# olga24912/lodestar

Hardware: AMD Instinct MI355X
Metric: verified signature sets/sec (node) (higher is better)
Workload: dtype u32/u64 (28-bit-limb Montgomery integer arithmetic); 1 GPU; C2 gossip attestation flood: 16384 single-pubkey sets per GPU, 1 set per batchable job; pk_mode=device table, sig_encoding=compressed 96 B, distinct_messages=16384, group_sets=1024, group_policy=0, inflight=32, slots=3, hw_queues=4, merge_sets=131072, pipeline_depth=3, parallelism=shard-by-job x1 (in-process devices), no collective

## Files before the change

### include/blsgpu.h

```cpp
#ifndef BLSGPU_H
#define BLSGPU_H

#include <stdint.h>

#ifdef __cplusplus
extern "C" {
#endif

#define BLSGPU_ABI_VERSION 8

#define BLSGPU_JOB_BATCHABLE 1u
#define BLSGPU_JOB_URGENT 2u

enum blsgpu_code {
  BLSGPU_OK = 0,
  BLSGPU_BAD_ENCODING = 1,
  BLSGPU_POINT_NOT_ON_CURVE = 2,
  BLSGPU_POINT_NOT_IN_GROUP = 3,
  BLSGPU_AGGR_TYPE_MISMATCH = 4,
  BLSGPU_VERIFY_FAIL = 5,
  BLSGPU_PK_IS_INFINITY = 6,
  BLSGPU_BAD_SCALAR = 7,
  BLSGPU_INVALID_SIZE = 8,
  BLSGPU_EMPTY_AGGREGATE = 9,
// ... 67 lines not shown
                                const uint8_t* sigs, uint32_t sig_stride, const uint32_t* sig_len,
                                uint32_t flags, uint8_t* out, uint32_t out_len, int8_t* status,
                                uint32_t* first_bad);
uint32_t blsgpu_sig_agg_lanes(uint32_t n_groups, uint32_t n_sigs);

int blsgpu_randomness_words(uint32_t n, uint64_t seed, uint64_t* words);

int blsgpu_aggregate_with_randomness(blsgpu_ctx* ctx, uint32_t n_groups, const uint32_t* group_first,
                                     const uint8_t* pk_bytes, const uint32_t* pk_index, const uint8_t* sigs,
                                     uint32_t sig_stride, const uint32_t* sig_len, uint64_t seed, uint8_t* out_pk,
                                     uint32_t out_pk_len, uint8_t* out_sig, uint32_t out_sig_len, int8_t* status,
                                     uint32_t* first_bad);
uint32_t blsgpu_awr_lanes(uint32_t n_groups, uint32_t n_sets);

#define BLSGPU_SAME_LANE_FORMS 1u

typedef struct blsgpu_same_message_stats {
  uint32_t groups_accepted;
  uint32_t groups_retried;
  uint32_t retry_sets;
  uint32_t unique_messages;
  uint32_t form;
  double device_ms;
} blsgpu_same_message_stats;

int blsgpu_verify_same_message(blsgpu_ctx* ctx, uint32_t n_groups, const uint32_t* group_first,
                               const uint8_t* msgs , const uint8_t* pk_bytes,
                               const uint32_t* pk_index, const uint8_t* sigs, uint32_t sig_stride,
                               const uint32_t* sig_len, uint64_t seed, uint32_t flags,
                               int8_t* set_result , int8_t* group_result ,
                               blsgpu_same_message_stats* stats );
uint32_t blsgpu_same_message_form(uint32_t n_items, uint32_t flags);

int blsgpu_key_validate(blsgpu_ctx* ctx, uint32_t n, const uint8_t* pks, uint32_t pk_len, uint32_t stride,
                        uint8_t* out96, int8_t* status);

#define BLSGPU_ROOT_OBJECT 0
#define BLSGPU_ROOT_ATTESTATION_DATA 1
int blsgpu_signing_roots(blsgpu_ctx* ctx, int kind, uint32_t n, const uint8_t* objects, uint32_t object_stride,
                         const uint8_t* domains, uint32_t domain_stride, uint8_t* out32);

int blsgpu_shard_jobs(const uint32_t* job_first_set, const uint32_t* set_pk_first, uint32_t n_jobs,
                      uint32_t n_parts, uint32_t* part_first_job);

int blsgpu_route_call(uint32_t n_sets, uint32_t n_devices, const int64_t* device_load, int64_t split_sets,
                      uint32_t start, uint32_t* out_devices, uint32_t* n_out);

int blsgpu_batch_scalars(const blsgpu_batch* b, uint64_t* words);

#define BLSGPU_INJECT_ENTROPY 1
#define BLSGPU_INJECT_DEVICE 2
int blsgpu_debug_inject(int what, int64_t skip, int64_t count);

const char* blsgpu_code_name(int code);

int blsgpu_debug_op(blsgpu_ctx* ctx, int op, uint32_t n, const uint8_t* in, uint32_t in_stride,
                    uint8_t* out, uint32_t out_stride, int32_t* status);

#ifdef __cplusplus
}
#endif
#endif
```

### lodestar_amd/csrc/k_miller.hip

```cpp
#include "k_common.hpp"
#include "gt_wave.hpp"
#include "gt6.hpp"
#include "gtx.hpp"

#ifndef BLS_LINE_PAIRS
#define BLS_LINE_PAIRS 0
#endif
#ifndef BLS_ACC2_PAIRS
#define BLS_ACC2_PAIRS 0
#endif

BLS_INL fp fp_add_n(const fp& a, const fp& b) { return fp_add_norm(a, b); }

#ifndef BLS_ACC_PREFETCH
#define BLS_ACC_PREFETCH 0
#endif
#if BLS_ACC_PREFETCH && defined(__HIP_DEVICE_COMPILE__)
#define LDS_AS __attribute__((address_space(3)))
__device__ __forceinline__ void line_prefetch(uint32_t* pre, const uint32_t* o, uint32_t nm, uint32_t m) {
  const uint32_t* a = o + opaque_u32(m);
#pragma unroll 1
  for (int w = 0; w < W_LINE; w++) {
    __builtin_amdgcn_global_load_lds((const void*)a, (LDS_AS void*)(pre + w * WAVE), 4, 0, 0);
    a += nm;
// ... 125 lines not shown
      line3 L;
      L.l0 = ld_fp2(o, b.nm, m, 0);
      L.c1 = ld_fp2(o, b.nm, m, 2 * W_FP);
      L.c4 = ld_fp2(o, b.nm, m, 4 * W_FP);
#endif
#if BLS_LINE_PAIRS
      const fp2 l1 = fp2_mul_fp(L.c1, P.x), l4 = fp2_mul_fp(L.c4, P.y);
      if (pend) {
        f = fp12_mul_by_line2(f, line_pair(q0, q1, q4, L.l0, l1, l4));
        pend = false;
      } else {
        q0 = L.l0;
        q1 = l1;
        q4 = l4;
        pend = true;
      }
#else
      f = fp12_mul_by_014(f, L.l0, fp2_mul_fp(L.c1, P.x), fp2_mul_fp(L.c4, P.y));
#endif
    }
#if BLS_LINE_PAIRS
    if (pend) f = fp12_mul_by_014(f, q0, q1, q4);
#endif
    if (!add_next) {
      add_next = (BLS_Z_ABS >> bit) & 1ull;
      bit--;
    } else {
      add_next = false;
    }
  }
  st_fp12(b.f_chunk, b.n, c, fp12_conj(f));
}

template <bool UNITS>
STAGE_KERNEL_W(BLSGPU_WPE_ACC) void k_miller_acc2(PipelineBuffers b) {
  const uint32_t q = blockIdx.x * WAVE + threadIdx.x;
  const uint32_t c = q >> 1, h = q & 1;
  if (c >= b.n_chunks) return;
  const uint32_t k0 = b.chunk_first[c], k1 = b.chunk_first[c + 1];
#if ACC_PREFETCH
  __shared__ uint32_t pre[W_LINE * WAVE];
  auto msg_of = [&](uint32_t k) {
    const uint32_t i = b.chunk_items[k];
    return UNITS ? b.unit_msg[i] : b.msg_idx[i];
  };
  if (k1 > k0) line_prefetch(pre, b.lines, b.nm, msg_of(k0));
#endif
  fp6 mine = h ? fp6_zero() : fp6_one();
  int bit = 62;
  bool add_next = false;
#pragma unroll 1
  for (int s = 0; s < MILLER_STEPS; s++) {
    if (!add_next && s != 0) {
      const fp6 other = fp6_xlane(mine);
      const fp6 a0 = h ? other : mine, a1 = h ? mine : other;
      fp6 X, Y;
      if (h) {
        X.c0 = fp2_make(fp_add_n(a0.c0.c0, a1.c0.c0), fp_add_n(a0.c0.c1, a1.c0.c1));
        X.c1 = fp2_make(fp_add_n(a0.c1.c0, a1.c1.c0), fp_add_n(a0.c1.c1, a1.c1.c1));
        X.c2 = fp2_make(fp_add_n(a0.c2.c0, a1.c2.c0), fp_add_n(a0.c2.c1, a1.c2.c1));
        Y.c0 = fp2_make(fp_lc(T<1>(a0.c0.c0), T<1>(a1.c2.c0), T<-1>(a1.c2.c1)),
                        fp_lc(T<1>(a0.c0.c1), T<1>(a1.c2.c0), T<1>(a1.c2.c1)));
        Y.c1 = fp2_make(fp_add_n(a0.c1.c0, a1.c0.c0), fp_add_n(a0.c1.c1, a1.c0.c1));
        Y.c2 = fp2_make(fp_add_n(a0.c2.c0, a1.c1.c0), fp_add_n(a0.c2.c1, a1.c1.c1));
      } else {
        X = a0;
        Y = a1;
      }
      const fp6 pr = fp6_mul(X, Y);
      const fp6 t = fp6_xlane(pr);
      fp6 r;
      if (h) {
        r.c0.c0 = fp_lc(T<1>(pr.c0.c0), T<-1>(t.c0.c0), T<-1>(t.c2.c0), T<1>(t.c2.c1));
        r.c0.c1 = fp_lc(T<1>(pr.c0.c1), T<-1>(t.c0.c1), T<-1>(t.c2.c0), T<-1>(t.c2.c1));
        r.c1.c0 = fp_lc(T<1>(pr.c1.c0), T<-1>(t.c1.c0), T<-1>(t.c0.c0));
        r.c1.c1 = fp_lc(T<1>(pr.c1.c1), T<-1>(t.c1.c1), T<-1>(t.c0.c1));
        r.c2.c0 = fp_lc(T<1>(pr.c2.c0), T<-1>(t.c2.c0), T<-1>(t.c1.c0));
        r.c2.c1 = fp_lc(T<1>(pr.c2.c1), T<-1>(t.c2.c1), T<-1>(t.c1.c1));
      } else {
        r.c0 = fp2_make(fp_lc(T<2>(pr.c0.c0)), fp_lc(T<2>(pr.c0.c1)));
        r.c1 = fp2_make(fp_lc(T<2>(pr.c1.c0)), fp_lc(T<2>(pr.c1.c1)));
        r.c2 = fp2_make(fp_lc(T<2>(pr.c2.c0)), fp_lc(T<2>(pr.c2.c1)));
      }
      mine = fp6_xlane(r);
    }
    const uint32_t* o = b.lines + (size_t)s * W_LINE * b.nm;
    auto fold = [&](const fp6& T0, const fp6& T1) {
      const fp6 T1v = h ? T1 : fp6_mul_v(T1);
      fp6 r;
      r.c0 = fp2_make(fp_lc(T<1>(T0.c0.c0), T<1>(T1v.c0.c0)), fp_lc(T<1>(T0.c0.c1), T<1>(T1v.c0.c1)));
      r.c1 = fp2_make(fp_lc(T<1>(T0.c1.c0), T<1>(T1v.c1.c0)), fp_lc(T<1>(T0.c1.c1), T<1>(T1v.c1.c1)));
      r.c2 = fp2_make(fp_lc(T<1>(T0.c2.c0), T<1>(T1v.c2.c0)), fp_lc(T<1>(T0.c2.c1), T<1>(T1v.c2.c1)));
      mine = r;
    };
#if BLS_ACC2_PAIRS
    bool pend = false;
    fp2 q0, q1, q4;
#endif
#pragma unroll 1
    for (uint32_t k = k0; k < k1; k++) {
      const uint32_t i = b.chunk_items[k];
      uint32_t m;
      bool active;
      if (UNITS) {
        m = b.unit_msg[i];
        active = b.unit_ok[i] != 0;
      } else {
        m = b.msg_idx[i];
        active = b.include[i] != 0;
      }
#if ACC_PREFETCH
      line_wait();
      fp2 l0 = ld_fp2_pre(pre, 0), l1 = ld_fp2_pre(pre, 2 * W_FP), l4 = ld_fp2_pre(pre, 4 * W_FP);
      line_read_done();
      if (k + 1 < k1)
        line_prefetch(pre, o, b.nm, msg_of(k + 1));
      else if (s + 1 < MILLER_STEPS)
        line_prefetch(pre, o + (size_t)W_LINE * b.nm, b.nm, msg_of(k0));
      if (!active || (b.mflags[m] & MF_H_INF)) continue;
      const g1a P = ld_g1a(UNITS ? b.unit_p : b.pk_aff, b.n, i);
      l1 = fp2_mul_fp(l1, P.x);
      l4 = fp2_mul_fp(l4, P.y);
#else
      if (!active || (b.mflags[m] & MF_H_INF)) continue;
      const g1a P = ld_g1a(UNITS ? b.unit_p : b.pk_aff, b.n, i);
      const fp2 l0 = ld_fp2(o, b.nm, m, 0);
      const fp2 l1 = fp2_mul_fp(ld_fp2(o, b.nm, m, 2 * W_FP), P.x);
      const fp2 l4 = fp2_mul_fp(ld_fp2(o, b.nm, m, 4 * W_FP), P.y);
#endif
#if BLS_ACC2_PAIRS
      if (!pend) {
        q0 = l0;
        q1 = l1;
        q4 = l4;
        pend = true;
        continue;
      }
      pend = false;
      const fp2 R1 = fp2_mul(h ? q4 : q0, h ? l4 : l0);
      const fp2 R2 = fp2_mul(h ? fp2_add_nr(q0, q4) : q1, h ? fp2_add_nr(l0, l4) : l1);
      const fp2 R3 = fp2_mul(h ? fp2_add_nr(q1, q4) : fp2_add_nr(q0, q1), h ? fp2_add_nr(l1, l4) : fp2_add_nr(l0, l1));
      const fp2 O1 = fp2_xlane(R1), O2 = fp2_xlane(R2), O3 = fp2_xlane(R3);
      const fp2 P00 = h ? O1 : R1, P44 = h ? R1 : O1, P11 = h ? O2 : R2, X04 = h ? R2 : O2, X01 = h ? O3 : R3,
                X14 = h ? R3 : O3;
      fp6 M0;
      M0.c0 = fp2_make(fp_lc(T<1>(P00.c0), T<1>(P44.c0), T<-1>(P44.c1)), fp_lc(T<1>(P00.c1), T<1>(P44.c0), T<1>(P44.c1)));
      M0.c1 = F2_LC3(X01, P00, P11);
      M0.c2 = P11;
      const fp2 m11 = F2_LC3(X04, P00, P44), m12 = F2_LC3(X14, P11, P44);
      const fp6 other = fp6_xlane(mine);
      fold(fp6_mul(mine, M0), fp6_mul_by_12(other, m11, m12));
#else
      const fp6 other = fp6_xlane(mine);
      fold(fp6_mul_by_01(mine, l0, l1), fp6_mul_by_1(other, l4));
#endif
    }
#if BLS_ACC2_PAIRS
    if (pend) {
      const fp6 other = fp6_xlane(mine);
      fold(fp6_mul_by_01(mine, q0, q1), fp6_mul_by_1(other, q4));
    }
#endif
// ... 190 lines not shown
```

### lodestar_amd/csrc/runtime.cpp

```cpp
#include <hip/hip_runtime.h>
#include <stdint.h>
#include <stdio.h>
#include <stdlib.h>
#include <string.h>
#include <pthread.h>
#include <sys/random.h>

#include <algorithm>
#include <cmath>
#include <atomic>
#include <chrono>
#include <condition_variable>
#include <deque>
#include <mutex>
#include <shared_mutex>
#include <string>
#include <system_error>
#include <thread>
#include <vector>

#include "../../include/blsgpu.h"
#include "batch_rand.hpp"
#include "kernels.h"

// ... 240 lines not shown
  int64_t fb_check6 = 2;
  int64_t keep_f = 1;
  int64_t keep_copy = 0;
  int64_t fb_force_busy = 0;
  int64_t urgent_lane = 1;
  int64_t urgent_max_sets = 512;
  int64_t urgent_excl = 0;
  int64_t urgent_wait_us = 300;
  int64_t group_adapt = 1;
  bool same_run(const struct Options& o) const {
    return group_sets == o.group_sets && profile == o.profile && dedupe == o.dedupe && miller_k == o.miller_k &&
           group_policy == o.group_policy && serial == o.serial && miller_lanes == o.miller_lanes &&
           f_run_max == o.f_run_max && lane_tail_min == o.lane_tail_min &&
           lane_tail_parts == o.lane_tail_parts &&
           msm_slice_mid == o.msm_slice_mid && msm_tree == o.msm_tree &&
           lines_lanes == o.lines_lanes && merge_balance == o.merge_balance && early_release == o.early_release && tail_on_msg == o.tail_on_msg && copy_stream == o.copy_stream && coop_max == o.coop_max &&
           coop_g2_max == o.coop_g2_max && coop_excl_max == o.coop_excl_max && rsig_spec == o.rsig_spec && spec_large == o.spec_large && spec_gsm == o.spec_gsm &&
           fb_lane_min == o.fb_lane_min && acc6_max == o.acc6_max && miller_pairs == o.miller_pairs && small_max == o.small_max &&
           fb_direct_min == o.fb_direct_min && fb_check6 == o.fb_check6 && fb_force_busy == o.fb_force_busy &&
           group_adapt == o.group_adapt && keep_f == o.keep_f && keep_copy == o.keep_copy;
  }
};

inline uint32_t chunk_size(uint32_t len, uint32_t min_per_chunk) {
  const uint32_t count = min_per_chunk ? len / min_per_chunk : 0;
  return count <= 1 ? len : (len + count - 1) / count;
}

struct GroupPlanEntry {
  uint32_t first, end;
  bool batchable;
};

inline uint32_t miller_k_auto(uint32_t n_items) {
  uint32_t k = 1;
  while (k < 4 && n_items / (2 * k) >= 65536) k *= 2;
  return k;
}

void launch_miller_acc_auto(const PipelineBuffers& pb, bool units, hipStream_t st, uint32_t mk, int64_t lanes_opt,
                            int64_t acc6_max, bool pairs) {
  if (lanes_opt == 6 || (lanes_opt == 0 && mk == 1 && (int64_t)pb.n_chunks <= acc6_max)) {
    launch_miller_acc6(pb, units, st);
    return;
  }
  if (lanes_opt == 3 || (lanes_opt == 0 && pairs)) {
    launch_miller_accx(pb, units, st);
    return;
  }
  const bool two = lanes_opt == 2 || (lanes_opt == 0 && mk == 1);
  if (two)
    launch_miller_acc2(pb, units, st);
  else
    launch_miller_acc(pb, units, st);
}

inline std::pair<uint32_t, uint32_t> add_chunks(std::vector<uint32_t>& first, std::vector<uint32_t>& items,
                                                uint32_t a, uint32_t e, uint32_t k, const uint32_t* map = nullptr) {
  const uint32_t c0 = (uint32_t)first.size() - 1;
  for (uint32_t x = a; x < e; x += k) {
    for (uint32_t y = x; y < std::min(e, x + k); y++) items.push_back(map ? map[y] : y);
    first.push_back((uint32_t)items.size());
  }
  return {c0, (uint32_t)first.size() - 1};
}

inline void add_slices(std::vector<uint32_t>& slices, std::vector<uint32_t>& range_slices, uint32_t a, uint32_t e,
                       uint32_t len = MSM_SLICE) {
  for (uint32_t x = a; x < e; x += len) {
    slices.push_back(x);
    slices.push_back(std::min<uint32_t>(e, x + len));
  }
  range_slices.push_back((uint32_t)(slices.size() / 2));
}

struct Shard {
  uint32_t job_begin, job_end;
  uint32_t set_begin, set_end;
  uint32_t dev = 0;
  int64_t cost = 0;
};

struct Owned {
  std::vector<uint32_t> jfs, siglen, pkfirst, pkidx;
  std::vector<uint8_t> jflags, pkb, msgs, sigs;
};

// ... 257 lines not shown
    std::vector<uint32_t> stamp(n_umsg, UINT32_MAX), unit_of_msg(n_umsg, 0);
    for (uint32_t g = 0; g < ng0; g++) {
      g_unit_first[g] = (uint32_t)unit_msg.size();
      const uint32_t a = job_sets(group_jobs[g].first).first, e = job_sets(group_jobs[g].second - 1).second;
      for (uint32_t i = a; i < e; i++) {
        const uint32_t m = msg_idx[i];
        if (stamp[m] != g) {
          stamp[m] = g;
          unit_of_msg[m] = (uint32_t)unit_msg.size();
          unit_msg.push_back(m);
        }
        unit_of_set[i] = unit_of_msg[m];
      }
    }
    g_unit_first[ng0] = (uint32_t)unit_msg.size();
    merged = unit_msg.size() < (size_t)n;
    if (merged) {
      const uint32_t nu = (uint32_t)unit_msg.size();
      unit_first.assign(nu + 1, 0);
      for (uint32_t i = 0; i < n; i++)
        if (unit_of_set[i] != UINT32_MAX) unit_first[unit_of_set[i] + 1]++;
      for (uint32_t u = 0; u < nu; u++) unit_first[u + 1] += unit_first[u];
      unit_sets.resize(unit_first[nu]);
      std::vector<uint32_t> fill(unit_first.begin(), unit_first.end() - 1);
      for (uint32_t i = 0; i < n; i++)
        if (unit_of_set[i] != UINT32_MAX) unit_sets[fill[unit_of_set[i]]++] = i;
    }
  }
  const uint32_t n_units = merged ? (uint32_t)unit_msg.size() : 0;
  const uint32_t n_items = merged ? n_units : n;
  const bool coop = n_items <= (uint32_t)opt.coop_max && opt.miller_k <= 1;
  const bool coop_g2 = n <= (uint32_t)opt.coop_g2_max;
  const bool excl = BLSGPU_EXCLUSIVE_SMALL && n_items <= (uint32_t)opt.coop_excl_max && (!sl.urgent || opt.urgent_excl);
  const uint32_t mk = coop ? 1u : opt.miller_k > 0 ? (uint32_t)opt.miller_k : miller_k_auto(n_items);
  std::vector<uint32_t> chunk_first{0}, chunk_items, g_chunks(2 * (size_t)ng0);
  chunk_items.reserve(n);
  for (uint32_t g = 0; g < ng0; g++) {
    const uint32_t a = merged ? g_unit_first[g] : job_sets(group_jobs[g].first).first;
    const uint32_t e = merged ? g_unit_first[g + 1] : job_sets(group_jobs[g].second - 1).second;
    const auto cr = add_chunks(chunk_first, chunk_items, a, e, mk);
    g_chunks[2 * g] = cr.first;
    g_chunks[2 * g + 1] = cr.second;
  }
  const uint32_t n_chunks = (uint32_t)chunk_first.size() - 1;
  const bool keep_f = opt.keep_f && !merged && mk == 1 && n_chunks == n;
  const bool small = n <= (uint32_t)opt.small_max;
  const bool spec = BLSGPU_STREAM_PAIRS && (small || opt.spec_large) && sl.alone && !opt.serial;
  const bool rsig_spec = spec && small && opt.rsig_spec;
  constexpr uint32_t kMsmHalfSliceMaxSets = 32768, kMsmSmallSliceMaxSets = 1024;
  const uint32_t slice_len = n <= kMsmSmallSliceMaxSets  ? 32
                             : n <= kMsmHalfSliceMaxSets ? (uint32_t)opt.msm_slice_mid
                                                         : MSM_SLICE;
  std::vector<uint32_t> slices, range_slices{0};
  uint32_t msm_tree = 0;
  for (uint32_t g = 0; g < ng0; g++)
    add_slices(slices, range_slices, job_sets(group_jobs[g].first).first, job_sets(group_jobs[g].second - 1).second,
               slice_len);
  const uint32_t n_slices = (uint32_t)(slices.size() / 2);
  if (n <= kMsmHalfSliceMaxSets && opt.msm_tree) {
    for (uint32_t g = 0; g < ng0; g++) msm_tree = std::max(msm_tree, range_slices[g + 1] - range_slices[g]);
    if ((uint64_t)ng0 * msm_tree > 2ull * n_slices) msm_tree = 0;
  }
  std::vector<uint32_t> ftree, f_level_end;
  uint32_t f_k = 1, f_max = 0;
  if (n_chunks > 16384)
    for (const uint32_t heads = opt.f_run_max > 16 ? 256u : 8192u;
         n_chunks / f_k > heads && f_k < (uint32_t)opt.f_run_max;)
// ... 231 lines not shown
    PipelineBuffers pbm = pb;
    if (spec) pbm.include = db + ob_spec;
    beg(0, s);
    launch_sig_decode(pb, n, s, coop_g2, spec ? sl.join_dec : nullptr, excl);
    end(0, s);
    const uint32_t* d_slices = reinterpret_cast<uint32_t*>(din + o_slices);
    const uint32_t* d_rslices = reinterpret_cast<uint32_t*>(din + o_rslices);
    if (rsig_spec) {
      HIPCHK(hipEventRecord(sl.join_rsig, s));
      HIPCHK(hipStreamWaitEvent(sp, sl.join_rsig, 0));
      PipelineBuffers pq = pb;
      pq.rsig = sl.d_fb.p;
      pq.scal_tab = sl.d_fb.p + (size_t)stride * W_G2J;
      launch_sig_scale(pq, n, sp);
      HIPCHK(hipEventRecord(sl.join_rsig, sp));
    }
    if (spec) {
      HIPCHK(hipStreamWaitEvent(smsm, sl.join_dec, 0));
      launch_spec_mask(pb, n, pbm.include, smsm);
      launch_sig_msm(pbm, d_slices, n_slices, d_rslices, ng0, sl.d_msmB.p, sl.d_msmW.p, sl.d_S.p, smsm, false,
                     msm_tree);
      HIPCHK(hipEventRecord(sl.join_msm, smsm));
    }
    HIPCHK(hipStreamWaitEvent(s, sl.join_pk, 0));
    beg(4, s);
    launch_job_mask(pb, s);
    HIPCHK(hipEventRecord(sl.join_mask, s));
    HIPCHK(hipStreamWaitEvent(sm, sl.join_mask, 0));
    beg(5, sm);
    if (merged) launch_unit_aggregate(pb, sm);
    if (coop)
      launch_miller_coop(pb, merged, sm, excl);
    else
      launch_miller_acc_auto(pb, merged, sm, mk, opt.miller_lanes, opt.acc6_max, opt.miller_pairs != 0);
    end(5, sm);
    if (keep_f && opt.keep_copy == 1)
      launch_copy_words(sl.d_fkeep.p, pb.f_chunk, (size_t)stride * W_FP12, sm);
    else if (keep_f)
      HIPCHK(hipMemcpyAsync(sl.d_fkeep.p, pb.f_chunk, (size_t)stride * W_FP12 * 4, hipMemcpyDeviceToDevice, sm));
    const uint32_t* d_franges = reinterpret_cast<uint32_t*>(din + o_franges);
    beg(6, sm);
    const uint32_t* d_ftree = reinterpret_cast<uint32_t*>(din + o_ftree);
    launch_group_tree(pb, d_franges, ng0, d_ftree, n_fruns, d_ftree + 2 * (size_t)n_fruns, f_level_end, sl.d_F.p, sm);
    end(6, sm);
    HIPCHK(hipEventRecord(sl.join_msg, sm));
    if (spec)
      HIPCHK(hipStreamWaitEvent(s, sl.join_msm, 0));
    else
      launch_sig_msm(pb, d_slices, n_slices, d_rslices, ng0, sl.d_msmB.p, sl.d_msmW.p, sl.d_S.p, s,
                     lane_tail && (opt.lane_tail_parts & 1), msm_tree);
    end(4, s);
    const bool tail_msg = opt.tail_on_msg && !opt.serial && BLSGPU_STREAM_PAIRS;
    hipStream_t sg = s;
    if (spec && opt.spec_gsm && !tail_msg) sg = smsm;
    if (tail_msg) {
      HIPCHK(hipEventRecord(sl.join_gsm, s));
      HIPCHK(hipStreamWaitEvent(sm, sl.join_gsm, 0));
      sg = stl = sm;
    }
    beg(kStages + 1, sg);
    launch_group_sig_miller(sl.d_S.p, ng0, sl.d_G.p, sg, excl && coop,
                            lane_tail && (opt.lane_tail_parts & 2));
    end(kStages + 1, sg);
    HIPCHK(hipEventRecord(sl.join_gsm, sg));
    HIPCHK(hipStreamWaitEvent(stl, sl.join_gsm, 0));
    HIPCHK(hipStreamWaitEvent(stl, sl.join_msg, 0));
    if (rsig_spec) HIPCHK(hipStreamWaitEvent(stl, sl.join_rsig, 0));
// ... 134 lines not shown
                 o_rset = o_rrs + rrs.size(), o_sub = o_rset + rset.size(), o_sel = o_sub + subr.size();
    const size_t words = o_sel + nr;
    sl.h_list.ensure(words);
    sl.d_list.ensure(words);
    uint32_t* hl = sl.h_list.p;
    memcpy(hl, rr.data(), rr.size() * 4);
    memcpy(hl + 2 * (size_t)nr, rf.data(), rf.size() * 4);
    memcpy(hl + 4 * (size_t)nr, rfirst.data(), rfirst.size() * 4);
    memcpy(hl + 4 * (size_t)nr + rfirst.size(), ritems.data(), ritems.size() * 4);
    memcpy(hl + o_rsl, rsl.data(), rsl.size() * 4);
    memcpy(hl + o_rrs, rrs.data(), rrs.size() * 4);
    memcpy(hl + o_rset, rset.data(), rset.size() * 4);
    if (nsub) memcpy(hl + o_sub, subr.data(), subr.size() * 4);
    sl.d_ok.ensure(nr + nsub);
    sl.h_ok.ensure(nr + nsub);
    sl.d_S.ensure((size_t)W_G2J * (nr + nsub));
    sl.d_F.ensure((size_t)W_FP12 * (nr + nsub));
    uint32_t* const dS = sl.d_S.p;
    uint32_t* const dF = sl.d_F.p;
    uint32_t* const dS_sub = sl.d_S.p + (size_t)W_G2J * nr;
    uint32_t* const dF_sub = sl.d_F.p + (size_t)W_FP12 * nr;
    HIPCHK(hipMemcpyAsync(sl.d_list.p, hl, o_sel * 4, hipMemcpyHostToDevice, sfb));
    PipelineBuffers pr = pb;
    pr.n_chunks = nc;
    pr.chunk_first = sl.d_list.p + 4 * (size_t)nr;
    pr.chunk_items = sl.d_list.p + 4 * (size_t)nr + rfirst.size();
    if (keep_f) {
      pr.f_chunk = sl.d_fkeep.p;
    } else {
      st.fallback_miller += (uint32_t)ritems.size();
      if (coop)
        launch_miller_coop(pr, false, sfb);
      else
        launch_miller_acc_auto(pr, false, sfb, mk, opt.miller_lanes, opt.acc6_max, opt.miller_pairs != 0);
    }
    st.fallback_jobs += nr;
    if (small_jobs) {
      if (!rsig_spec) sl.d_fb.ensure((size_t)stride * 9 * W_G2J);
      pr.rsig = sl.d_fb.p;
      pr.scal_tab = sl.d_fb.p + (size_t)stride * W_G2J;
      if (!rsig_spec) launch_sig_scale(pr, (uint32_t)rset.size(), sfb, sl.d_list.p + o_rset);
      launch_group_reduce_lane(pr, sl.d_list.p, sl.d_list.p + 2 * (size_t)nr, nr, dS, dF, sfb);
    } else {
      sl.d_msmB.ensure((size_t)MSM_BUCKET_WORDS * std::max<uint32_t>(nrs, 1));
      sl.d_msmW.ensure((size_t)MSM_WINDOW_WORDS * nr);
      launch_sig_msm(pr, sl.d_list.p + o_rsl, nrs, sl.d_list.p + o_rrs, nr, sl.d_msmB.p, sl.d_msmW.p, dS, sfb);
      launch_group_reduce(pr, sl.d_list.p + 2 * (size_t)nr, nr, dF, sfb);
    }
    std::vector<uint32_t> sel;
    if (nsub) {
      if (nsub >= kFbLaneMin)
        launch_range_combine_lane(dS, dF, nr, sl.d_list.p + o_sub, nsub, dS_sub, dF_sub, sfb);
      else
        launch_range_combine(dS, dF, nr, sl.d_list.p + o_sub, nsub, dS_sub, dF_sub, sfb);
      fb_check(dS_sub, dF_sub, nsub, sl.d_ok.p + nr, nullptr, nsub);
      HIPCHK(hipGetLastError());
      HIPCHK(hipMemcpyAsync(sl.h_ok.p + nr, sl.d_ok.p + nr, nsub, hipMemcpyDeviceToHost, sfb));
      HIPCHK(hipEventRecord(sl.done, sfb));
      HIPCHK(hipEventSynchronize(sl.done));
      for (uint32_t t = 0; t < nsub; t++)
        for (uint32_t q = subr[2 * t]; q < subr[2 * t + 1]; q++) {
          if (sl.h_ok.p[nr + t]) jr[retry[q]] = 1;
          else sel.push_back(q);
        }
    } else {
      for (uint32_t q = 0; q < nr; q++) sel.push_back(q);
    }
// ... 1705 lines not shown
      ab.sig_flags = pb.flags;
      ab.sig_status = pb.status;
      ab.tab = sl.d_work.p + (size_t)n * W_G2A;
      ab.tab_n = lanes;
      ab.sum_pk = ab.tab + (size_t)lanes * AWR_TAB_WORDS;
      ab.sum_sig = ab.sum_pk + (size_t)G * W_G1J;
      ab.err_k = reinterpret_cast<uint32_t*>(din + o_ek);
      ab.err_c = reinterpret_cast<int8_t*>(din + o_ec);
      int8_t* d_gst = reinterpret_cast<int8_t*>(din + o_gst);
      uint32_t* d_fb = reinterpret_cast<uint32_t*>(din + o_fb);
      launch_sig_decode(pb, n, s, n <= 4096, nullptr, false, true);
      launch_awr_sums(ab, L, s);
      launch_awr_serialize(ab, din + o_opk, out_pk_len, din + o_osig, out_sig_len, d_gst, d_fb, s);
      HIPCHK(hipGetLastError());
      HIPCHK(hipMemcpyAsync(out_pk, din + o_opk, (size_t)G * out_pk_len, hipMemcpyDeviceToHost, s));
      HIPCHK(hipMemcpyAsync(out_sig, din + o_osig, (size_t)G * out_sig_len, hipMemcpyDeviceToHost, s));
      HIPCHK(hipMemcpyAsync(status, din + o_gst, G, hipMemcpyDeviceToHost, s));
      if (first_bad) HIPCHK(hipMemcpyAsync(first_bad, din + o_fb, (size_t)G * 4, hipMemcpyDeviceToHost, s));
      HIPCHK(hipStreamSynchronize(s));
    }
  } catch (HipError&) {
    rc = BLSGPU_DEVICE_ERROR;
  }
  leave(ctx);
  return rc;
}

uint32_t blsgpu_awr_lanes(uint32_t n_groups, uint32_t n_sets) { return awr_lanes(n_groups, n_sets); }

constexpr uint32_t kSameCoopMax = 512;
uint32_t blsgpu_same_message_form(uint32_t n_items, uint32_t flags) {
  return (flags & BLSGPU_SAME_LANE_FORMS) || n_items > kSameCoopMax ? 1u : 0u;
}
namespace {
inline bool same_serial() {
  static const bool on = [] {
    const char* v = getenv("BLSGPU_SAME_SERIAL");
    return v && v[0] == '1';
  }();
  return on;
}
void same_pairing_phase(const PipelineBuffers& pm, uint32_t n_items, const uint32_t* iota, uint32_t* pk_aff,
                        uint8_t* include, const uint32_t* msg_idx, const uint32_t* S, uint32_t* F, uint32_t* Gs,
                        uint8_t* ok, bool lane, hipStream_t s) {
  PipelineBuffers pb = pm;
  pb.n = n_items;
  pb.pk_aff = pk_aff;
  pb.include = include;
  pb.msg_idx = msg_idx;
  pb.n_chunks = n_items;
  pb.chunk_first = iota;
  pb.chunk_items = iota;
  pb.f_chunk = F;
  if (!lane) {
    launch_miller_coop(pb, false, s, false);
    launch_group_check(S, F, n_items, ok, s);
  } else {
    launch_miller_acc6(pb, false, s);
    launch_group_sig_miller(S, n_items, Gs, s, false, true);
    launch_group_check6(F, Gs, n_items, ok, s);
  }
}
}

int blsgpu_verify_same_message(blsgpu_ctx* ctx, uint32_t n_groups, const uint32_t* group_first, const uint8_t* msgs,
                               const uint8_t* pk_bytes, const uint32_t* pk_index, const uint8_t* sigs,
// ... 351 lines not shown
```

### lodestar_amd/native.py

```python
import ctypes
import os

import numpy as np

PKG = os.path.dirname(os.path.abspath(__file__))
LIB_PATH = os.environ.get("BLSGPU_LIB") or os.path.join(PKG, "libblsgpu.so")

OK = 0
BAD_ENCODING = 1
POINT_NOT_ON_CURVE = 2
POINT_NOT_IN_GROUP = 3
PK_IS_INFINITY = 6
INVALID_SIZE = 8
EMPTY_AGGREGATE = 9
EMPTY_SET = 10
DEVICE_ERROR = 11
ERR_ARGS = 100
ERR_NO_DEVICE = 101
ERR_CLOSED = 102
ERR_ENTROPY = 103
JOB_BATCHABLE = 1
JOB_URGENT = 2
AGG_VALIDATE = 1
AGG_MAX_SIGS = 1 << 20
INJECT_ENTROPY = 1
INJECT_DEVICE = 2

EXPORTED_SYMBOLS = [
    "blsgpu_init",
    "blsgpu_destroy",
    "blsgpu_device_count",
    "blsgpu_pubkeys_upload",
    "blsgpu_pubkeys_count",
    "blsgpu_verify",
    "blsgpu_submit",
    "blsgpu_set_option",
    "blsgpu_code_name",
    "blsgpu_debug_op",
    "blsgpu_aggregate_pubkeys",
    "blsgpu_key_validate",
    "blsgpu_signing_roots",
    "blsgpu_shard_jobs",
    "blsgpu_get_option",
    "blsgpu_chunkify",
    "blsgpu_batch_scalars",
    "blsgpu_debug_inject",
    "blsgpu_route_call",
    "blsgpu_aggregate_signatures",
    "blsgpu_sig_agg_lanes",
    "blsgpu_randomness_words",
    "blsgpu_aggregate_with_randomness",
    "blsgpu_awr_lanes",
    "blsgpu_verify_same_message",
    "blsgpu_same_message_form",
]
SAME_LANE_FORMS = 1
ROOT_OBJECT = 0
ROOT_ATTESTATION_DATA = 1


class Batch(ctypes.Structure):
    _fields_ = [
        ("n_sets", ctypes.c_uint32),
        ("n_jobs", ctypes.c_uint32),
        ("job_first_set", ctypes.c_void_p),
        ("job_flags", ctypes.c_void_p),
        ("pk_bytes", ctypes.c_void_p),
        ("set_pk_first", ctypes.c_void_p),
        ("pk_index", ctypes.c_void_p),
        ("msgs", ctypes.c_void_p),
        ("sigs", ctypes.c_void_p),
        ("sig_len", ctypes.c_void_p),
        ("sig_stride", ctypes.c_uint32),
        ("seed", ctypes.c_uint64),
    ]


class Stats(ctypes.Structure):
    _fields_ = [
        ("groups", ctypes.c_uint32),
        ("batch_retries", ctypes.c_uint32),
        ("batch_sigs_success", ctypes.c_uint32),
        ("devices_used", ctypes.c_uint32),
        ("device_ms", ctypes.c_double),
        ("stage_ms", ctypes.c_double * 8),
        ("unique_messages", ctypes.c_uint32),
        ("pairing_units", ctypes.c_uint32),
# ... 64 lines not shown
    lib.blsgpu_code_name.argtypes = [ctypes.c_int]
    lib.blsgpu_code_name.restype = ctypes.c_char_p
    lib.blsgpu_debug_op.argtypes = [ctypes.c_void_p, ctypes.c_int, ctypes.c_uint32, ctypes.c_void_p, ctypes.c_uint32,
                                    ctypes.c_void_p, ctypes.c_uint32, ctypes.c_void_p]
    lib.blsgpu_debug_op.restype = ctypes.c_int
    vp, u32 = ctypes.c_void_p, ctypes.c_uint32
    lib.blsgpu_aggregate_pubkeys.argtypes = [vp, ctypes.POINTER(Batch), vp, u32, vp]
    lib.blsgpu_key_validate.argtypes = [vp, u32, vp, u32, u32, vp, vp]
    lib.blsgpu_signing_roots.argtypes = [vp, ctypes.c_int, u32, vp, u32, vp, u32, vp]
    lib.blsgpu_shard_jobs.argtypes = [vp, vp, u32, u32, vp]
    lib.blsgpu_get_option.argtypes = [vp, ctypes.c_char_p, ctypes.POINTER(ctypes.c_int64)]
    lib.blsgpu_chunkify.argtypes = [u32, u32, vp, vp]
    lib.blsgpu_batch_scalars.argtypes = [ctypes.POINTER(Batch), vp]
    lib.blsgpu_batch_scalars.restype = ctypes.c_int
    lib.blsgpu_debug_inject.argtypes = [ctypes.c_int, ctypes.c_int64, ctypes.c_int64]
    lib.blsgpu_debug_inject.restype = ctypes.c_int
    lib.blsgpu_route_call.argtypes = [u32, u32, vp, ctypes.c_int64, u32, vp, vp]
    lib.blsgpu_route_call.restype = ctypes.c_int
    lib.blsgpu_aggregate_signatures.argtypes = [vp, u32, vp, vp, u32, vp, u32, vp, u32, vp, vp]
    lib.blsgpu_aggregate_signatures.restype = ctypes.c_int
    lib.blsgpu_sig_agg_lanes.argtypes = [u32, u32]
    lib.blsgpu_sig_agg_lanes.restype = u32
    lib.blsgpu_randomness_words.argtypes = [u32, ctypes.c_uint64, vp]
    lib.blsgpu_randomness_words.restype = ctypes.c_int
    lib.blsgpu_aggregate_with_randomness.argtypes = [vp, u32, vp, vp, vp, vp, u32, vp, ctypes.c_uint64, vp, u32, vp,
                                                     u32, vp, vp]
    lib.blsgpu_aggregate_with_randomness.restype = ctypes.c_int
    lib.blsgpu_awr_lanes.argtypes = [u32, u32]
    lib.blsgpu_awr_lanes.restype = u32
    lib.blsgpu_verify_same_message.argtypes = [vp, u32, vp, vp, vp, vp, vp, u32, vp, ctypes.c_uint64, u32, vp, vp, vp]
    lib.blsgpu_verify_same_message.restype = ctypes.c_int
    lib.blsgpu_same_message_form.argtypes = [u32, u32]
    lib.blsgpu_same_message_form.restype = u32
    _lib = lib
    return lib


def code_name(code: int) -> str:
    n = load().blsgpu_code_name(code)
    return n.decode() if n else f"BLSGPU_{code}"


def shard_jobs(job_first_set, n_parts, set_pk_first=None):
    jfs = np.ascontiguousarray(job_first_set, dtype=np.uint32)
    spf = None if set_pk_first is None else np.ascontiguousarray(set_pk_first, dtype=np.uint32)
    out = np.zeros(n_parts + 1, np.uint32)
    rc = load().blsgpu_shard_jobs(jfs.ctypes.data, None if spf is None else spf.ctypes.data, len(jfs) - 1, n_parts,
                                  out.ctypes.data)
    if rc != OK:
        raise ValueError(f"blsgpu_shard_jobs -> {code_name(rc)}")
    return [(int(out[k]), int(out[k + 1])) for k in range(n_parts)]


def route_call(n_sets, device_load, split_sets=16384, start=0):
    dl = np.ascontiguousarray(device_load, dtype=np.int64)
    out = np.zeros(max(len(dl), 1), np.uint32)
    k = ctypes.c_uint32(0)
    rc = load().blsgpu_route_call(n_sets, len(dl), dl.ctypes.data, split_sets, start, out.ctypes.data,
                                  ctypes.addressof(k))
    if rc != OK:
        raise ValueError(f"blsgpu_route_call -> {code_name(rc)}")
    return [int(x) for x in out[: k.value]]


def sig_agg_lanes(n_groups, n_sigs):
    return int(load().blsgpu_sig_agg_lanes(n_groups, n_sigs))
# ... 2 lines not shown
def aggregate_layout(sigs, group_first, sig_len=None, sig_stride=None, out_len=96):
    gf = np.ascontiguousarray(group_first, dtype=np.int64)
    if gf.ndim != 1 or len(gf) == 0:
        raise ValueError("group_first needs n_groups + 1 >= 1 entries")
    if gf[0] != 0 or (np.diff(gf) < 0).any():
        raise ValueError("group_first must start at 0 and never decrease")
    n = int(gf[-1])
    if n > AGG_MAX_SIGS:
        raise ValueError(f"at most {AGG_MAX_SIGS} signatures per call")
    if out_len not in (96, 192):
        raise ValueError("out_len must be 96 or 192")
    buf = _u8(sigs)
    if sig_stride is None:
        sig_stride = (len(buf) // n) if n else 96
    if sig_stride < 96:
        raise ValueError("sig_stride must be at least 96")
    if len(buf) < n * sig_stride:
        raise ValueError(f"{n} signatures of stride {sig_stride} need {n * sig_stride} bytes, got {len(buf)}")
    sl = np.full(n, sig_stride if sig_stride in (96, 192) else 96, np.uint32) if sig_len is None else \
        np.ascontiguousarray(sig_len, dtype=np.uint32)
    if sl.ndim != 1 or len(sl) != n:
        raise ValueError(f"sig_len needs one entry per signature ({n})")
    if sig_stride < 192 and (sl == 192).any():
        raise ValueError("a 192-byte signature needs sig_stride >= 192")
    return buf, gf.astype(np.uint32), sl, int(sig_stride)


def awr_lanes(n_groups, n_sets):
    return int(load().blsgpu_awr_lanes(n_groups, n_sets))


def same_message_form(n_items, flags=0):
    return int(load().blsgpu_same_message_form(n_items, flags))


def randomness_words(n, seed):
    out = np.zeros(max(n, 1), np.uint64)
    rc = load().blsgpu_randomness_words(n, seed, out.ctypes.data)
    if rc != OK:
        raise RuntimeError(f"blsgpu_randomness_words -> {code_name(rc)}")
    return out[:n]


def awr_layout(group_first, sigs, pk_bytes=None, pk_index=None, sig_len=None, sig_stride=None, out_pk_len=96,
               out_sig_len=192):
    if out_pk_len not in (48, 96):
        raise ValueError("out_pk_len must be 48 or 96")
    buf, gf, sl, stride = aggregate_layout(sigs, group_first, sig_len, sig_stride, out_sig_len)
    n = int(gf[-1])
    if (pk_bytes is None) == (pk_index is None):
        raise ValueError("exactly one of pk_bytes and pk_index")
    pkb = pki = None
    if pk_bytes is not None:
        pkb = _u8(pk_bytes)
        if len(pkb) != 96 * n:
            raise ValueError(f"{n} sets need {96 * n} pubkey bytes, got {len(pkb)}")
    else:
        idx = np.ascontiguousarray(pk_index, dtype=np.int64)
        if idx.ndim != 1 or len(idx) != n:
            raise ValueError(f"pk_index needs one entry per set ({n})")
        if n and (idx.min() < 0 or idx.max() > 0xFFFFFFFF):
            raise ValueError("pk_index entries must be table indices")
        pki = idx.astype(np.uint32)
    return gf, buf, sl, stride, pkb, pki


# ... 294 lines not shown
```

Measured before the change: 3.909 million sets/s.

## Split acc2 line scaling across lane pair and prefetch chunk item lookups

In the two-lane Miller accumulation kernel, each lane of a pair now loads only one pubkey coordinate and one line coefficient, scales it, and swaps the result with its partner via a cross-lane exchange. Before, both lanes loaded both coordinates and did both multiplies. The first few chunk items are looked up into registers up front, along with their message indices and skip flags. The runtime heuristic also picks miller_k=2 for large item counts when no lane option is set, and a new API reports which form is chosen. The lane exchange adds cross-lane traffic and the held-item arrays add register pressure.

```diff
diff --git a/include/blsgpu.h b/include/blsgpu.h
--- a/include/blsgpu.h
+++ b/include/blsgpu.h
@@ -123,6 +123,8 @@
                                blsgpu_same_message_stats* stats );
 uint32_t blsgpu_same_message_form(uint32_t n_items, uint32_t flags);
 
+uint32_t blsgpu_miller_form(uint32_t n_items, uint32_t miller_k, uint32_t miller_lanes);
+
 int blsgpu_key_validate(blsgpu_ctx* ctx, uint32_t n, const uint8_t* pks, uint32_t pk_len, uint32_t stride,
                         uint8_t* out96, int8_t* status);
 
diff --git a/lodestar_amd/csrc/k_miller.hip b/lodestar_amd/csrc/k_miller.hip
--- a/lodestar_amd/csrc/k_miller.hip
+++ b/lodestar_amd/csrc/k_miller.hip
@@ -181,20 +181,50 @@
   st_fp12(b.f_chunk, b.n, c, fp12_conj(f));
 }
 
+#ifndef ACC2_HOLD
+#define ACC2_HOLD 4
+#endif
 template <bool UNITS>
 STAGE_KERNEL_W(BLSGPU_WPE_ACC) void k_miller_acc2(PipelineBuffers b) {
   const uint32_t q = blockIdx.x * WAVE + threadIdx.x;
   const uint32_t c = q >> 1, h = q & 1;
   if (c >= b.n_chunks) return;
   const uint32_t k0 = b.chunk_first[c], k1 = b.chunk_first[c + 1];
+  uint32_t hold_i[ACC2_HOLD ? ACC2_HOLD : 1], hold_m[ACC2_HOLD ? ACC2_HOLD : 1], skip = 0;
+  auto lookup = [&](uint32_t k, uint32_t& i, uint32_t& m) {
+    i = b.chunk_items[k];
+    m = UNITS ? b.unit_msg[i] : b.msg_idx[i];
+    const bool active = (UNITS ? b.unit_ok[i] : b.include[i]) != 0;
+    return active && !(b.mflags[m] & MF_H_INF);
+  };
+#pragma unroll
+  for (uint32_t j = 0; j < ACC2_HOLD; j++) {
+    hold_i[j] = hold_m[j] = 0;
+    if (k0 + j < k1 && !lookup(k0 + j, hold_i[j], hold_m[j])) skip |= 1u << j;
+  }
+  auto item = [&](uint32_t k, uint32_t& i, uint32_t& m) {
+    const uint32_t j = k - k0;
+    if (j >= ACC2_HOLD) return lookup(k, i, m);
+    i = hold_i[0];
+    m = hold_m[0];
+#pragma unroll
+    for (uint32_t t = 1; t < ACC2_HOLD; t++) {
+      i = j == t ? hold_i[t] : i;
+      m = j == t ? hold_m[t] : m;
+    }
+    return !((skip >> j) & 1u);
+  };
 #if ACC_PREFETCH
   __shared__ uint32_t pre[W_LINE * WAVE];
   auto msg_of = [&](uint32_t k) {
-    const uint32_t i = b.chunk_items[k];
-    return UNITS ? b.unit_msg[i] : b.msg_idx[i];
+    uint32_t i, m;
+    item(k, i, m);
+    return m;
   };
   if (k1 > k0) line_prefetch(pre, b.lines, b.nm, msg_of(k0));
 #endif
+  const size_t own_line = (size_t)((2 + 2 * h) * W_FP) * b.nm;
+  const uint32_t* const own_p = (UNITS ? b.unit_p : b.pk_aff) + (size_t)(h * W_FP) * b.n;
   fp6 mine = h ? fp6_zero() : fp6_one();
   int bit = 62;
   bool add_next = false;
@@ -248,35 +278,24 @@
 #endif
 #pragma unroll 1
     for (uint32_t k = k0; k < k1; k++) {
-      const uint32_t i = b.chunk_items[k];
-      uint32_t m;
-      bool active;
-      if (UNITS) {
-        m = b.unit_msg[i];
-        active = b.unit_ok[i] != 0;
-      } else {
-        m = b.msg_idx[i];
-        active = b.include[i] != 0;
-      }
+      uint32_t i, m;
+      const bool active = item(k, i, m);
 #if ACC_PREFETCH
       line_wait();
-      fp2 l0 = ld_fp2_pre(pre, 0), l1 = ld_fp2_pre(pre, 2 * W_FP), l4 = ld_fp2_pre(pre, 4 * W_FP);
+      const fp2 l0 = ld_fp2_pre(pre, 0), cq = ld_fp2_pre(pre, (int)((2 + 2 * h) * W_FP));
       line_read_done();
       if (k + 1 < k1)
         line_prefetch(pre, o, b.nm, msg_of(k + 1));
       else if (s + 1 < MILLER_STEPS)
         line_prefetch(pre, o + (size_t)W_LINE * b.nm, b.nm, msg_of(k0));
-      if (!active || (b.mflags[m] & MF_H_INF)) continue;
-      const g1a P = ld_g1a(UNITS ? b.unit_p : b.pk_aff, b.n, i);
-      l1 = fp2_mul_fp(l1, P.x);
-      l4 = fp2_mul_fp(l4, P.y);
+      if (!active) continue;
 #else
-      if (!active || (b.mflags[m] & MF_H_INF)) continue;
-      const g1a P = ld_g1a(UNITS ? b.unit_p : b.pk_aff, b.n, i);
-      const fp2 l0 = ld_fp2(o, b.nm, m, 0);
-      const fp2 l1 = fp2_mul_fp(ld_fp2(o, b.nm, m, 2 * W_FP), P.x);
-      const fp2 l4 = fp2_mul_fp(ld_fp2(o, b.nm, m, 4 * W_FP), P.y);
-#endif
+      if (!active) continue;
+      const fp2 l0 = ld_fp2(o, b.nm, m, 0), cq = ld_fp2(o + own_line, b.nm, m, 0);
+#endif
+      const fp2 sc = fp2_mul_fp(cq, ld_fp(own_p, b.n, i, 0));
+      const fp2 sx = fp2_xlane(sc);
+      const fp2 l1 = h ? sx : sc, l4 = h ? sc : sx;
 #if BLS_ACC2_PAIRS
       if (!pend) {
         q0 = l0;
diff --git a/lodestar_amd/csrc/runtime.cpp b/lodestar_amd/csrc/runtime.cpp
--- a/lodestar_amd/csrc/runtime.cpp
+++ b/lodestar_amd/csrc/runtime.cpp
@@ -296,27 +296,29 @@
   bool batchable;
 };
 
-inline uint32_t miller_k_auto(uint32_t n_items) {
+inline uint32_t miller_k_auto(uint32_t n_items, int64_t lanes_opt, bool pairs) {
   uint32_t k = 1;
   while (k < 4 && n_items / (2 * k) >= 65536) k *= 2;
+  if (k == 1 && lanes_opt == 0 && !pairs && n_items >= 65536) k = 2;
   return k;
 }
 
-void launch_miller_acc_auto(const PipelineBuffers& pb, bool units, hipStream_t st, uint32_t mk, int64_t lanes_opt,
-                            int64_t acc6_max, bool pairs) {
-  if (lanes_opt == 6 || (lanes_opt == 0 && mk == 1 && (int64_t)pb.n_chunks <= acc6_max)) {
-    launch_miller_acc6(pb, units, st);
-    return;
-  }
-  if (lanes_opt == 3 || (lanes_opt == 0 && pairs)) {
-    launch_miller_accx(pb, units, st);
-    return;
-  }
-  const bool two = lanes_opt == 2 || (lanes_opt == 0 && mk == 1);
-  if (two)
-    launch_miller_acc2(pb, units, st);
-  else
-    launch_miller_acc(pb, units, st);
+inline uint32_t miller_lanes_pick(uint32_t mk, uint32_t n_items, uint32_t n_chunks, int64_t lanes_opt,
+                                  int64_t acc6_max, bool pairs) {
+  if (lanes_opt == 6 || (lanes_opt == 0 && mk == 1 && (int64_t)n_chunks <= acc6_max)) return 6;
+  if (lanes_opt == 3 || (lanes_opt == 0 && pairs)) return 3;
+  if (lanes_opt) return lanes_opt == 1 ? 1 : 2;
+  return mk > 1 && n_items / mk >= 65536 ? 1 : 2;
+}
+
+void launch_miller_acc_auto(const PipelineBuffers& pb, bool units, hipStream_t st, uint32_t mk, uint32_t n_items,
+                            int64_t lanes_opt, int64_t acc6_max, bool pairs) {
+  switch (miller_lanes_pick(mk, n_items, pb.n_chunks, lanes_opt, acc6_max, pairs)) {
+    case 6: launch_miller_acc6(pb, units, st); break;
+    case 3: launch_miller_accx(pb, units, st); break;
+    case 2: launch_miller_acc2(pb, units, st); break;
+    default: launch_miller_acc(pb, units, st);
+  }
 }
 
 inline std::pair<uint32_t, uint32_t> add_chunks(std::vector<uint32_t>& first, std::vector<uint32_t>& items,
@@ -640,7 +642,8 @@
   const bool coop = n_items <= (uint32_t)opt.coop_max && opt.miller_k <= 1;
   const bool coop_g2 = n <= (uint32_t)opt.coop_g2_max;
   const bool excl = BLSGPU_EXCLUSIVE_SMALL && n_items <= (uint32_t)opt.coop_excl_max && (!sl.urgent || opt.urgent_excl);
-  const uint32_t mk = coop ? 1u : opt.miller_k > 0 ? (uint32_t)opt.miller_k : miller_k_auto(n_items);
+  const uint32_t mk = coop ? 1u : opt.miller_k > 0 ? (uint32_t)opt.miller_k
+                                                   : miller_k_auto(n_items, opt.miller_lanes, opt.miller_pairs != 0);
   std::vector<uint32_t> chunk_first{0}, chunk_items, g_chunks(2 * (size_t)ng0);
   chunk_items.reserve(n);
   for (uint32_t g = 0; g < ng0; g++) {
@@ -938,7 +941,7 @@
     if (coop)
       launch_miller_coop(pb, merged, sm, excl);
     else
-      launch_miller_acc_auto(pb, merged, sm, mk, opt.miller_lanes, opt.acc6_max, opt.miller_pairs != 0);
+      launch_miller_acc_auto(pb, merged, sm, mk, n_items, opt.miller_lanes, opt.acc6_max, opt.miller_pairs != 0);
     end(5, sm);
     if (keep_f && opt.keep_copy == 1)
       launch_copy_words(sl.d_fkeep.p, pb.f_chunk, (size_t)stride * W_FP12, sm);
@@ -1139,7 +1142,7 @@
       if (coop)
         launch_miller_coop(pr, false, sfb);
       else
-        launch_miller_acc_auto(pr, false, sfb, mk, opt.miller_lanes, opt.acc6_max, opt.miller_pairs != 0);
+        launch_miller_acc_auto(pr, false, sfb, mk, (uint32_t)ritems.size(), opt.miller_lanes, opt.acc6_max, opt.miller_pairs != 0);
     }
     st.fallback_jobs += nr;
     if (small_jobs) {
@@ -2911,6 +2914,13 @@
 uint32_t blsgpu_same_message_form(uint32_t n_items, uint32_t flags) {
   return (flags & BLSGPU_SAME_LANE_FORMS) || n_items > kSameCoopMax ? 1u : 0u;
 }
+uint32_t blsgpu_miller_form(uint32_t n_items, uint32_t miller_k, uint32_t miller_lanes) {
+  const Options def;
+  const bool pairs = def.miller_pairs != 0;
+  const uint32_t mk = miller_k ? miller_k : miller_k_auto(n_items, miller_lanes, pairs);
+  const uint32_t n_chunks = (n_items + mk - 1) / mk;
+  return 256 * mk + miller_lanes_pick(mk, n_items, n_chunks, miller_lanes, def.acc6_max, pairs);
+}
 namespace {
 inline bool same_serial() {
   static const bool on = [] {
diff --git a/lodestar_amd/native.py b/lodestar_amd/native.py
--- a/lodestar_amd/native.py
+++ b/lodestar_amd/native.py
@@ -53,6 +53,7 @@
     "blsgpu_awr_lanes",
     "blsgpu_verify_same_message",
     "blsgpu_same_message_form",
+    "blsgpu_miller_form",
 ]
 SAME_LANE_FORMS = 1
 ROOT_OBJECT = 0
@@ -183,6 +184,8 @@
     lib.blsgpu_verify_same_message.restype = ctypes.c_int
     lib.blsgpu_same_message_form.argtypes = [u32, u32]
     lib.blsgpu_same_message_form.restype = u32
+    lib.blsgpu_miller_form.argtypes = [u32, u32, u32]
+    lib.blsgpu_miller_form.restype = u32
     _lib = lib
     return lib
 
@@ -251,6 +254,11 @@
 
 def same_message_form(n_items, flags=0):
     return int(load().blsgpu_same_message_form(n_items, flags))
+
+
+def miller_form(n_items, miller_k=0, miller_lanes=0):
+    v = int(load().blsgpu_miller_form(n_items, miller_k, miller_lanes))
+    return v >> 8, v & 255
 
 
 def randomness_words(n, seed):
```

Result: no change. 3.909 million sets/s (-0.0%).
